# articulatory/articulatory

Hardware: AMD Instinct MI355X
Metric: audio samples/sec (16 kHz) EMA->wav HiFi-CAR, batch 64 (higher is better)
Workload: dtype fp32; 1 GPU; configs[2]: HiFi-CAR (e2w_hifigan_car.yaml generator) 13-dim pitch+EMA -> 16 kHz, batch 64/GPU, 10 s clips, 80 sequential chunks of 25 frames; batch_per_gpu=64, frames=2000, chunk_frames=25, weights=synthetic seed 1234 (articulatory_amd.utils.synth), parallelism=utterance-sharded x1, arithmetic=exact fp32 products (v_mfma_f32_32x32x2_f32), fp32 accumulate, gather=none

## Files before the change

### __graft_entry__.py

```python

import os
import subprocess
import sys

REPO = os.path.dirname(os.path.abspath(__file__))
if REPO not in sys.path:
    sys.path.insert(0, REPO)


def build() -> None:
    csrc = os.path.join(REPO, "articulatory_amd", "csrc")
    subprocess.run(["make", "-C", csrc, f"-j{max(1, min(14, os.cpu_count() or 1))}"], check=True)
    import articulatory_amd
    from articulatory_amd import _native

    lib = _native.load_library()
    for sym in _native.SYMBOLS:
        getattr(lib, sym)
    print("built", _native.LIB_PATH, lib.hificar_version().decode())


def smoke() -> None:
    import numpy as np
    import torch

    from articulatory_amd.models import HiFiGANGenerator
    from articulatory_amd.utils.synth import synth_features, synth_state_dict
# ... 47 lines not shown
```

### articulatory_amd/csrc/hificar.hip

```cpp
#include "hificar_kernels.hip.h"
#include "hificar_launch.h"
#include "hificar_backward.hip.h"
#include "hificar_disc_kernels.hip.h"
#include "hificar_bigru_kernels.hip.h"
#include "hificar_bigru_train_kernels.hip.h"
#include "hificar_xfmr_kernels.hip.h"
#include "hificar_xfmr_attn16.hip.h"
#include "hificar_xfmr_train_kernels.hip.h"
#include "hificar_xfmr_attn16_train.hip.h"
#include "hificar_xfmr_wgrad16.hip.h"

#include "../../include/hificar.h"

#include <algorithm>
#include <queue>
#include <set>
#include <cmath>
#include <cstdarg>
#include <cstdio>
#include <cstring>
#include <functional>
#include <map>
#include <memory>
#include <string>
// ... 51 lines not shown
};

struct PlanKey {
    const ConvLayer* layers[6];
    int nseq, rows, zrep;
    int flags;
    bool operator<(const PlanKey& o) const { return memcmp(this, &o, sizeof(PlanKey)) < 0; }
};

struct ConvPlan {
    ConvShape shape;
    unsigned grid = 0;
    size_t lds = 0;
    std::string name;
    MultiConvParams conv = {};
    PairParams pair = {};
    MergeConvParams merge = {};
    bool merge_wins = false;
};

struct hificar_engine {
    int precision = HIFICAR_PREC_F32;
    int num_cus = 256;
    bool training = false;
    bool profile_detail = false;
    bool use_pair = true;
    bool pair_small = true;
    int mrf_merge = 1;
    int ksplit = 1;
    double mi1_penalty = 1.05;
    int pick_throughput = 0;
    bool shared_chip = false;
    int force_tile[5] = {0, 0, 0, 0, 0};
    std::vector<void*> allocs;
    char* d_zeros = nullptr;
    std::map<PlanKey, ConvPlan> plans;
    struct Arena {
        char* d = nullptr;
        char* h = nullptr;
        size_t cap = 0, used = 0;
    };
    std::vector<Arena> arenas;
    unsigned long long sched_up_seq = 0;
// ... 77 lines not shown
    float* tap_scratch = nullptr;
    size_t tap_scratch_elems = 0;
};

static FILE* g_launch_log = nullptr;
static void read_env_switches(hificar_engine* h) {
    if (const char* e = getenv("HIFICAR_PROFILE_DETAIL")) h->profile_detail = atoi(e) != 0;
    if (const char* e = getenv("HIFICAR_LAUNCH_LOG")) {
        if (!g_launch_log && *e) g_launch_log = fopen(e, "a");
        if (g_launch_log) h->profile_detail = true;
    }
    if (const char* e = getenv("HIFICAR_KSPLIT")) h->ksplit = atoi(e);
    if (const char* e = getenv("HIFICAR_PAIR")) h->use_pair = atoi(e) != 0;
    if (const char* e = getenv("HIFICAR_PAIR_SMALL")) h->pair_small = atoi(e) != 0;
    if (const char* e = getenv("HIFICAR_MRF_MERGE")) h->mrf_merge = atoi(e);
}

struct ProfScope {
    hificar_engine* h;
    hipStream_t s;
    hipEvent_t e0 = nullptr, e1 = nullptr;
    std::string name;
    double flops, bytes;
    ProfScope(hificar_engine* h_, hipStream_t s_, const std::string& n, double f, double b) : h(h_), s(s_), flops(f), bytes(b) {
        if (g_launch_log) {
            fprintf(g_launch_log, "%s\t%.0f\t%.0f\n", n.c_str(), f, b);
            fflush(g_launch_log);
        }
        if (!h->profiling) return;
        name = n;
// ... 359 lines not shown
    if (!L.transposed && L.cin_pad == L.cin && (L.cin == 32 || L.cin == 64) && L.cout == L.cin) {
        if ((rc = pack_w16(h, L, W, L.cin_pad, &L.d_w16c)) != HIFICAR_OK) return rc;
        if ((rc = pack_w32(h, L, W, L.cin_pad, &L.d_w32c)) != HIFICAR_OK) return rc;
    }
    return HIFICAR_OK;
}

hipError_t hificar::conv_launch(const ConvShape& s, const void* params, dim3 grid, size_t lds_bytes, hipStream_t stream) {
    bool handled = false;
    hipError_t e = hipSuccess;
#define HIFICAR_TRY_SET(n)                                                      \
    if (!handled) e = conv_inst_launch_##n(s, params, grid, lds_bytes, stream, &handled); \
    if (handled) return e;
    HIFICAR_TRY_SET(0) HIFICAR_TRY_SET(1) HIFICAR_TRY_SET(2) HIFICAR_TRY_SET(3) HIFICAR_TRY_SET(4)
    HIFICAR_TRY_SET(5) HIFICAR_TRY_SET(6) HIFICAR_TRY_SET(7) HIFICAR_TRY_SET(8) HIFICAR_TRY_SET(9)
    HIFICAR_TRY_SET(10) HIFICAR_TRY_SET(11) HIFICAR_TRY_SET(12)
#undef HIFICAR_TRY_SET
    return hipErrorInvalidValue;
}

hipError_t hificar::conv_set_lds_attributes() {
    hipError_t e = hipSuccess;
#define HIFICAR_ATTR_SET(n) \
    if (e == hipSuccess) e = conv_inst_attrs_##n();
    HIFICAR_ATTR_SET(0) HIFICAR_ATTR_SET(1) HIFICAR_ATTR_SET(2) HIFICAR_ATTR_SET(3) HIFICAR_ATTR_SET(4)
    HIFICAR_ATTR_SET(5) HIFICAR_ATTR_SET(6) HIFICAR_ATTR_SET(7) HIFICAR_ATTR_SET(8) HIFICAR_ATTR_SET(9)
    HIFICAR_ATTR_SET(10) HIFICAR_ATTR_SET(11) HIFICAR_ATTR_SET(12)
#undef HIFICAR_ATTR_SET
    return e;
}

static int engine_open(hificar_engine* h, bool read_env) {
    int dev = 0;
    hipDeviceProp_t prop;
    if (hipGetDevice(&dev) == hipSuccess && hipGetDeviceProperties(&prop, dev) == hipSuccess && prop.multiProcessorCount > 0)
        h->num_cus = prop.multiProcessorCount;
    if (read_env) read_env_switches(h);
    void* z = nullptr;
    HIP_TRY(hipMalloc(&z, 256));
    h->allocs.push_back(z);
    HIP_TRY(hipMemset(z, 0, 256));
    h->d_zeros = static_cast<char*>(z);
// ... 365 lines not shown
            if (!h->xstream_ev) HIP_TRY(hipEventCreateWithFlags(&h->xstream_ev, hipEventDisableTiming));
            HIP_TRY(hipEventRecord(h->xstream_ev, h->last_stream));
            HIP_TRY(hipStreamWaitEvent(stream, h->xstream_ev, 0));
        }
    }
    h->done_valid = false;
    h->last_stream = stream;
    h->have_last_stream = true;
    return HIFICAR_OK;
}

struct TileCfg {
    int MI, WM, WN;
    int KS;
    int NB;
};
static size_t out_buf_bytes(const TileCfg& t) { return (size_t)t.KS * (t.WM * t.MI * 32) * (t.WN * t.NB * 32 + 4) * sizeof(float); }
constexpr int kNumTileCfgs = 15;
static const TileCfg kTileCfgs[kNumTileCfgs] = {{4, 1, 4, 1, 1}, {4, 2, 2, 1, 1}, {4, 4, 1, 1, 1}, {2, 2, 2, 1, 2}, {2, 4, 1, 1, 2},
                                                {2, 1, 4, 1, 2}, {2, 1, 4, 1, 1}, {2, 2, 2, 1, 1}, {2, 4, 1, 1, 1},
                                                {1, 1, 4, 1, 1}, {1, 2, 2, 1, 1}, {1, 4, 1, 1, 1}, {4, 1, 1, 4, 1}, {2, 1, 1, 4, 1}, {1, 1, 1, 4, 1}};

struct ConvIO {
    const char* xs;
    const float* res;
    float* y;
    char* ys;
    const float* mask_src = nullptr;
    float mask_slope = 0.f;
    long long x_seq_bytes = 0;
    int x_row_bytes = 0;
    int x_rows = 0;
    int x_up = 0;
    float x_slope = -1.f;
    const float* x_more[3] = {nullptr, nullptr, nullptr};
    int x_n = 1;
    bool res_relu = false;
};

struct ConvRep {
    int n = 1;
    long long zs_x = 0, zs_w = 0, zs_y = 0, zs_b = 0;
};

static bool tile_admissible(const hificar_engine* h, const ConvLayer* const* layers, int nbr, const TileCfg& t, int halo_all, int nsteps_min) {
    const ConvLayer& L0 = *layers[0];
    const bool f32 = h->precision == HIFICAR_PREC_F32;
    const int TM = t.WM * t.MI * 32, RB = L0.chunk16 * 4;
    if (t.NB == 2 && (f32 || L0.chunk16 == 16)) return false;
    const size_t obuf = (f32 && t.KS == 1) ? 0 : out_buf_bytes(t);
    if (2 * round_up_sz((size_t)(TM + halo_all) * RB, 1024) + obuf > 160 * 1024) return false;
    if (t.NB == 2) {
        bool ok = L0.n_blocks32 >= 2;
        for (int b = 0; b < nbr; ++b) ok = ok && (layers[b]->n_phase == 1 || layers[b]->nb32_per_phase % 2 == 0);
        if (!ok) return false;
    }
    if (t.KS == 4 && (h->ksplit == 0 || nsteps_min < 2)) return false;
    return true;
}

static TileCfg pick_tile(const hificar_engine* h, const ConvLayer* const* layers, int nbr, int nseq, int rows, int zrep, bool merged = false,
                         double* est = nullptr, bool use_force = true) {
    const ConvLayer& L0 = *layers[0];
    const bool f32 = h->precision == HIFICAR_PREC_F32;
    int halo_all = 0;
    for (int b = 0; b < nbr; ++b) halo_all = std::max(halo_all, layers[b]->off_max - layers[b]->off_min);
    TileCfg tc = {1, 4, 1, 1, 1};
    double best = 1e300;
    int nsteps_min = 1 << 30;
    for (int b = 0; b < nbr; ++b) nsteps_min = std::min(nsteps_min, layers[b]->ntaps * (L0.chunk16 / 16));
    if (h->force_tile[0] != 0 && use_force) {
        const TileCfg t = {h->force_tile[0], h->force_tile[1], h->force_tile[2], h->force_tile[3], h->force_tile[4]};
        if (tile_admissible(h, layers, nbr, t, halo_all, nsteps_min) && (!merged || (t.KS == 1 && t.NB == 1))) return t;
    }
    for (int ti = 0; ti < kNumTileCfgs; ++ti) {
        const TileCfg& t = kTileCfgs[ti];
        const int TM = t.WM * t.MI * 32;
        const int chunk = L0.chunk16;
        if (!tile_admissible(h, layers, nbr, t, halo_all, nsteps_min)) continue;
        if (merged && (t.KS != 1 || t.NB != 1)) continue;
        if (!merged && t.KS == 1 && h->ksplit == 2 && nsteps_min >= 2) continue;
        const long long tiles_per_branch = (long long)nseq * ((rows + TM - 1) / TM) * ((L0.n_blocks32 + t.WN * t.NB - 1) / (t.WN * t.NB));
        const int ncls = merged ? 1 : nbr;
        const long long total = tiles_per_branch * ncls * zrep;
        const int G = (int)std::min<long long>(total, h->num_cus);
        const int nchunks = L0.cin_pad / chunk;
        double total_cost = 0.0, heaviest = 0.0, lightest = 1e300, cb[3] = {0.0, 0.0, 0.0};
        for (int b = 0; b < nbr; ++b) {
            const double slab = f32 ? 8 * 64.0 : 3 * 32 / 0.75;
            double c = (double)layers[b]->ntaps * (L0.cin_pad / 16) * slab * t.MI * t.NB + 2500.0 + 400.0 * nchunks;
            if (t.KS == 4) {
                const int steps = layers[b]->ntaps * (chunk / 16);
                c = (double)((steps + 3) / 4) * nchunks * slab * t.MI + 4000.0 + 600.0 * nchunks;
            }
            if (merged) {
                cb[0] += c - (b ? 2500.0 : 0.0);
                continue;
// ... 26 lines not shown
        if (h->pick_throughput > 0 && total >= h->pick_throughput) worst = total_cost / h->num_cus;
        if (t.NB == 2) worst *= f32 ? (t.MI == 4 ? 0.95 : t.MI == 2 ? 0.975 : 1.02) : (t.MI == 2 ? 0.93 : 1.10);
        else if (t.MI < 4) worst *= f32 ? (t.MI == 2 ? 1.02 : h->mi1_penalty) : (t.MI == 2 ? 1.10 : 1.25);
        if (t.KS == 4) worst *= 1.05;
        if (worst < best * 0.98) {
            best = worst;
            tc = t;
        }
    }
    if (est) *est = best;
    return tc;
}

static std::string plan_name(const hificar_engine* h, const ConvShape& s, const ConvLayer& L0, int nbr) {
    static const char* const family[] = {"conv_f32do_kernel", "conv_bf16x3_kernel", "conv_bf16x3nb_kernel", "conv_sk_f32_kernel", "conv_sk_bf16x3_kernel",
                                         "conv_pair_f32_kernel", "conv_pair_bf16x3_kernel", "conv_f32mrg_kernel"};
    char kname[96];
    int n = s.family == kConvSkF32 || s.family == kConvSkBf16x3 ? snprintf(kname, sizeof(kname), "%s<%d,%d>", family[s.family], s.mi, s.nc16)
                                                                : snprintf(kname, sizeof(kname), "%s<%d,%d,%d,%d>", family[s.family], s.mi, s.wm, s.wn, s.nc16);
    if (h->profile_detail) snprintf(kname + n, sizeof(kname) - n, s.family == kConvF32mrg ? "|%s +%d" : "|%s x%d", L0.name.c_str(), nbr);
    return kname;
}

static int build_conv_plan(hificar_engine* h, const ConvLayer* const* layers, int nbr, int nseq, int rows, int zrep, hipStream_t stream, ConvPlan& pl) {
    const ConvLayer& L0 = *layers[0];
    const bool f32 = h->precision == HIFICAR_PREC_F32;
    MultiConvParams& mp = pl.conv;
    const TileCfg tc = pick_tile(h, layers, nbr, nseq, rows, zrep);
    int halo_all = 0;
    for (int b = 0; b < nbr; ++b) halo_all = std::max(halo_all, layers[b]->off_max - layers[b]->off_min);
    const int TM = tc.WM * tc.MI * 32, nc16 = L0.chunk16 / 16;
    const size_t buf_bytes = round_up_sz((size_t)(TM + halo_all) * L0.chunk16 * 4, 1024);
    const bool dout = f32 && tc.KS == 1;
    pl.shape = {dout ? kConvF32do : tc.KS == 4 ? (f32 ? kConvSkF32 : kConvSkBf16x3) : tc.NB == 2 ? kConvBf16x3nb : kConvBf16x3, tc.MI, tc.WM, tc.WN, nc16};
    pl.lds = 2 * buf_bytes + (dout ? 0 : out_buf_bytes(tc));
    mp.buf_bytes = (int)buf_bytes;
    mp.n_branches = nbr;
    mp.nseq_tiles = nseq * ((rows + TM - 1) / TM);
    mp.ngroups = (L0.n_blocks32 + tc.WN * tc.NB - 1) / (tc.WN * tc.NB);
    mp.total_tiles = nbr * zrep * mp.ngroups * mp.nseq_tiles;
    pl.grid = (unsigned)std::min(mp.total_tiles, h->num_cus);
    {
        double wbytes = 0.0;
        for (int b = 0; b < nbr; ++b) wbytes += 4.0 * layers[b]->cin_pad * layers[b]->cout_total * layers[b]->ntaps * zrep;
        const double abytes = 4.0 * nseq * rows * L0.cin_pad * nbr * zrep;
        mp.xcd_order = (mp.total_tiles <= h->num_cus && mp.total_tiles >= 16 && wbytes > 2.0 * abytes) ? 1 : 0;
    }
    mp.stage_cached = mp.ngroups > 2 ? 1 : 0;
    pl.name = plan_name(h, pl.shape, L0, nbr);
    TileLists lists;
    if (mp.total_tiles <= h->num_cus && nbr == 1 && zrep == 1 && mp.ngroups >= 2 && mp.nseq_tiles >= 8 && !h->shared_chip &&
        4.0 * L0.cin_pad * L0.cout_total * L0.ntaps > 6.0e6)
        lists = xcd_block_lists(mp.nseq_tiles, mp.ngroups, h->num_cus);
// ... 103 lines not shown
    pp.in_bytes = (int)round_up_sz((size_t)(TMc + halo_max) * RB, 1024);
    pp.ts_bytes = (int)std::max<size_t>((size_t)(TMc + 16) * RB, (size_t)TMc * (C + 4) * sizeof(float));
    pl.lds = (size_t)pp.in_bytes + pp.ts_bytes;
    if (pl.lds > 160 * 1024) return fail(HIFICAR_E_INVALID, "internal: pair kernel LDS too large (%zu)", pl.lds);
    pl.grid = (unsigned)std::min(tile, h->num_cus);
    pl.shape = {f32 ? kPairF32 : kPairBf16x3, MI, WM, 4 / WM, C / 16};
    pl.name = plan_name(h, pl.shape, *l1[0], nbr);
    if (tile <= (int)pl.grid) return HIFICAR_OK;
    std::vector<double> costs((size_t)tile);
    for (int b = 0; b < nbr; ++b)
        for (int i = pp.tile_start[b]; i < pp.tile_start[b + 1]; ++i) costs[i] = l1[b]->ntaps + l2[b]->ntaps + 2.0;
    return upload_schedule(h, lpt_lists(costs, (int)pl.grid), tile, stream, &pp.sched_start, &pp.sched_tiles);
}

static const ConvPlan* get_plan(hificar_engine* h, const ConvLayer* const* a, const ConvLayer* const* b, int nbr, int nseq, int rows, int zrep,
                                hipStream_t stream, int* rc, bool merged = false) {
    *rc = HIFICAR_OK;
    PlanKey k = {{}, nseq, rows, zrep, (h->precision == HIFICAR_PREC_F32 ? 1 : 0) | (h->training ? 2 : 0) | (h->shared_chip ? 4 : 0) | (b ? 8 : 0) | (merged ? 16 : 0)};
    for (int i = 0; i < nbr; ++i) k.layers[i] = a[i];
    for (int i = 0; b && i < nbr; ++i) k.layers[3 + i] = b[i];
    auto it = h->plans.find(k);
    if (it == h->plans.end()) {
        ConvPlan pl;
        if (h->plans.size() > 20000) *rc = evict_plans(h);
        if (*rc == HIFICAR_OK)
            *rc = merged ? build_merge_plan(h, a, nbr, nseq, rows, stream, pl)
                  : b    ? build_pair_plan(h, a, b, nbr, nseq, rows, stream, pl)
                         : build_conv_plan(h, a, nbr, nseq, rows, zrep, stream, pl);
        if (*rc != HIFICAR_OK) return nullptr;
        it = h->plans.emplace(k, std::move(pl)).first;
    }
    return &it->second;
}

static int launch_conv(hificar_engine* h, const ConvLayer* const* layers, int nbr, int nseq, int rows, const ConvIO* io,
                              float slope_out, const Ragged& rg, hipStream_t stream, const ConvRep& zr = ConvRep()) {
    int rc;
    const ConvPlan* const pl = get_plan(h, layers, nullptr, nbr, nseq, rows, zr.n, stream, &rc);
    if (!pl) return rc;
    const int TM = pl->shape.wm * pl->shape.mi * 32;
    const ConvLayer& L0 = *layers[0];
    const bool f32 = h->precision == HIFICAR_PREC_F32;
    MultiConvParams mp = pl->conv;
    double flops = 0.0, bytes = 0.0;
    for (int b = 0; b < nbr; ++b) {
        const ConvLayer& Lb = *layers[b];
        if (Lb.n_blocks32 != L0.n_blocks32 || Lb.chunk16 != L0.chunk16 || Lb.cin_pad != L0.cin_pad)
            return fail(HIFICAR_E_INVALID, "internal: branch shape mismatch");
        fill_params(mp.p[b], Lb, rows, TM, io[b].res, io[b].y, rg);
        mp.p[b].xs = io[b].xs;
        mp.p[b].ys = io[b].ys;
        if (io[b].x_slope >= 0.f) {
            if (!f32) return fail(HIFICAR_E_INVALID, "internal: pre-activation input rows of %s outside the exact-fp32 layer-by-layer launches", Lb.name.c_str());
            if (io[b].x_n < 1 || io[b].x_n > 4) return fail(HIFICAR_E_INVALID, "internal: %d input streams of %s", io[b].x_n, Lb.name.c_str());
            mp.p[b].act_in = io[b].x_n;
            for (int q = 0; q + 1 < io[b].x_n; ++q) mp.p[b].xs_more[q] = reinterpret_cast<const char*>(io[b].x_more[q]);
            mp.p[b].slope_in = io[b].x_slope;
        }
        if (io[b].res_relu) {
            if (f32 || pl->shape.family == kConvSkBf16x3)
                return fail(HIFICAR_E_INVALID, "internal: pre-activation residual rows of %s outside the dense bf16x3 launches", Lb.name.c_str());
            mp.p[b].res_relu = 1;
        }
        mp.p[b].mask_src = io[b].mask_src;
// ... 11 lines not shown
        mp.p[b].zeros = h->d_zeros;
        mp.p[b].slope_out = slope_out;
        mp.p[b].cout_real = Lb.cout_pad;
        if (f32) mp.p[b].w16 = reinterpret_cast<const bf16x8*>(Lb.d_w32);
        const double pos = (double)nseq * rows;
        flops += 2.0 * pos * Lb.cin * Lb.cout * Lb.K * zr.n;
        bytes += 4.0 * (pos * Lb.cin_pad * (io[b].x_slope >= 0.f ? io[b].x_n : 1) / std::max(1, io[b].x_up) + pos * Lb.cout_total * ((io[b].res ? 1 : 0) + (io[b].y ? 1 : 0) + (io[b].ys ? 1 : 0)) +
                        (double)Lb.cin * Lb.cout * Lb.K);
    }
    mp.zrep = zr.n;
    mp.zs_x = zr.zs_x;
    mp.zs_w = zr.zs_w;
    mp.zs_y = zr.zs_y;
    mp.zs_b = zr.zs_b;
    ProfScope prof(h, stream, pl->name, flops, bytes);
    const hipError_t e = conv_launch(pl->shape, &mp, dim3(pl->grid, 1, 1), pl->lds, stream);
    if (e != hipSuccess) return fail(HIFICAR_E_HIP, "conv launch (%s, %s) failed: %s", L0.name.c_str(), pl->name.c_str(), hipGetErrorString(e));
    return HIFICAR_OK;
}

static int launch_merged(hificar_engine* h, const ConvPlan* pl, const ConvLayer* const* layers, int nbr, int nseq, int rows, const ConvIO* io, char* ys_out,
                         float slope_out, const Ragged& rg, hipStream_t stream) {
    const int TM = pl->shape.wm * pl->shape.mi * 32;
    const ConvLayer& L0 = *layers[0];
    MergeConvParams mp = pl->merge;
    double flops = 0.0, bytes = 0.0;
    const double pos = (double)nseq * rows;
    for (int b = 0; b < nbr; ++b) {
        const ConvLayer& Lb = *layers[b];
        if (Lb.n_blocks32 != L0.n_blocks32 || Lb.chunk16 != L0.chunk16 || Lb.cin_pad != L0.cin_pad || Lb.cout_total != L0.cout_total || Lb.n_phase != 1 ||
            !io[b].res || !io[b].xs || io[b].xs == ys_out)
// ... 962 lines not shown
```

### articulatory_amd/csrc/hificar_conv.hip.h

```cpp
#pragma once
#include <hip/hip_runtime.h>
#include <stdint.h>
#include <type_traits>

namespace hificar {

typedef float f32x2 __attribute__((ext_vector_type(2)));
typedef float f32x4 __attribute__((ext_vector_type(4)));
typedef unsigned u32x4_t __attribute__((ext_vector_type(4)));
typedef float f32x16 __attribute__((ext_vector_type(16)));
typedef __bf16 bf16x4 __attribute__((ext_vector_type(4)));
typedef __bf16 bf16x8 __attribute__((ext_vector_type(8)));

constexpr int kMaxPhase = 8;
constexpr int kMaxTaps = 16;

struct ConvParams {
    const bf16x8* w16;
    const float* bias;
    const float* res;
    const float* mask_src;
    float mask_slope;
    float* y;
    const float* xf;
// ... 28 lines not shown
};

__device__ __forceinline__ int scalar_load_i32(const int* p) {
    int v;
    asm volatile("s_load_dword %0, %1, 0x0\n\ts_waitcnt lgkmcnt(0)" : "=s"(v) : "s"(p) : "memory");
    return v;
}

__device__ __forceinline__ void scalar_load_2i32(const int* p, int& a, int& b) {
    long long v;
    asm volatile("s_load_dwordx2 %0, %1, 0x0\n\ts_waitcnt lgkmcnt(0)" : "=s"(v) : "s"(p) : "memory");
    a = (int)v;
    b = (int)(v >> 32);
}

__device__ __forceinline__ bool is_ragged(const ConvParams& p) { return p.seq_len != nullptr || p.len_const >= 0; }

__device__ __forceinline__ int seq_rows(const ConvParams& p, int seq) {
    if (!is_ragged(p)) return p.L;
    const int n = (p.seq_len ? scalar_load_i32(p.seq_len + __builtin_amdgcn_readfirstlane(seq)) : p.len_const) - p.len_f0;
    return min(max(n, 0), p.len_max) * p.len_mul;
}

template <int NBR>
struct MultiConvParamsN {
    ConvParams p[NBR];
    int n_branches;
    int nseq_tiles;
    int ngroups;
    int total_tiles;
    int buf_bytes;
    const int* sched_start;
    const int* sched_tiles;
    int zrep;
    long long zs_x, zs_w, zs_y, zs_b;
    unsigned long long* trace;
    int xcd_order;
    int stage_cached;
};
struct MultiConvParams : MultiConvParamsN<3> {};
struct MergeConvParams : MultiConvParamsN<4> {};


#ifdef HIFICAR_TRACE
__device__ unsigned long long g_trace_realtime[2][1024];
__device__ unsigned long long g_trace_rt_slots[4][64];
#define HIFICAR_STAMP(slot)                                                                            \
    do {                                                                                               \
        if (mp.trace && lane == 0 && (wave == 0 || wave == kFirstLoader) && (slot) < 64)               \
            mp.trace[((size_t)blockIdx.x * 2 + (wave ? 1 : 0)) * 64 + (slot)] = __builtin_amdgcn_s_memtime(); \
        if (mp.trace && lane == 0 && wave == 0 && ((slot) == 0 || (slot) == 63) && blockIdx.x < 1024)  \
            g_trace_realtime[(slot) == 63][blockIdx.x] = __builtin_amdgcn_s_memrealtime();             \
        if (mp.trace && lane == 0 && wave == 0 && (slot) < 64 && blockIdx.x < 4)                       \
            g_trace_rt_slots[blockIdx.x][(slot)] = __builtin_amdgcn_s_memrealtime();                   \
    } while (0)
// ... 11 lines not shown
        constexpr int lo = NMEM * I / NMFMA, hi = NMEM * (I + 1) / NMFMA;
        constexpr int ds = (hi < NDS ? hi : NDS) - (lo < NDS ? lo : NDS);
        constexpr int vm = (hi - lo) - ds;
        __builtin_amdgcn_sched_group_barrier(0x008, 1, 0);
        if constexpr (ds > 0) __builtin_amdgcn_sched_group_barrier(0x100, ds, 0);
        if constexpr (vm > 0) __builtin_amdgcn_sched_group_barrier(0x020, vm, 0);
        pin_slab_slot<I + 1, NDS, NVMEM, NMFMA>();
    }
}
template <int NDS, int NVMEM, int NMFMA>
__device__ __forceinline__ void pin_slab_step() {
    pin_slab_slot<0, NDS, NVMEM, NMFMA>();
}
__device__ __forceinline__ void lds_barrier() { asm volatile("s_waitcnt lgkmcnt(0)\n\ts_barrier" ::: "memory"); }

template <int MI, int WM, int WN, int NC16, bool F32, int KS = 1, int NB = 1, bool DOUT = false, bool MRG = false, class MP = MultiConvParams>
__device__ __forceinline__ void conv_ws_body(const MP& mp) {
    static_assert(!DOUT || (F32 && KS == 1 && NB == 1), "direct output: exact fp32, dense form, one channel block per wave");
    static_assert(!MRG || DOUT, "branch-summing form: a direct-output kernel");
    static_assert(NB == 1 || (NB == 2 && KS == 1), "one or two channel blocks per MFMA wave");
    static_assert(KS == 1 || (KS == 4 && WM == 1 && WN == 1), "split-K: four waves share one 32-channel block");
    static_assert(KS == 4 || WM * WN == 4 || WM * WN == 8, "4 or 8 MFMA waves per workgroup");
    constexpr int NW = KS == 4 ? 4 : WM * WN;
    constexpr bool kPrimeOnce = DOUT;
    constexpr bool kRowMajorAcc = DOUT;
    constexpr int NTHR = (NW + 4) * 64;
    constexpr int kFirstLoader = NW;
    (void)kFirstLoader;
    static_assert(NC16 == 1 || NC16 == 2 || NC16 == 4, "chunk of 16, 32 or 64 channels");
    constexpr int TM = WM * MI * 32;
    constexpr int CH = NC16 * 16;
    constexpr int RB = CH * 4;
    constexpr int SPR = CH / 4;
    constexpr int LOG_SPR = NC16 == 4 ? 4 : NC16 == 2 ? 3 : 2;
// ... 171 lines not shown
        }
    };
    if (loader) {
        const int lw = wave - NW;
        const int ltid = tid - NW * 64;

        auto dma_item = [&](const Tile& T, int c, int jj) {
            const ConvParams& p = mp.p[T.b];
            const int R = TM + p.halo;
            const int ninstr = (R * SPR + 63) >> 6;
            const int Ls = p.x_rows ? p.x_rows : seq_rows(p, T.seq);
            const int row_bytes = p.x_row_bytes ? p.x_row_bytes : p.cin * 4;
            const char* const xs_z = p.xs + (size_t)T.z * mp.zs_x + (size_t)T.seq * (p.x_seq_bytes ? (size_t)p.x_seq_bytes : (size_t)p.L * p.cin * 4);
            char* dst = smem_b + (jj & 1) * buf_bytes;
            const int c0b = c * CH * 2;
            for (int i = lw; i < ninstr; i += 4) {
                const int n = i * 64 + lane;
                const int r = n >> LOG_SPR;
                const int sl = (n & (SPR - 1)) ^ ((r >> LOG_RPB) & (SPR - 1));
                const int t = T.t0 + p.off_min + r;
                const char* src = p.zeros;
                if (r < R && t >= 0 && t < Ls) {
                    const int ts = p.x_up > 1 ? (int)__umulhi((unsigned)t, p.x_up_rcp) : t;
                    if constexpr (F32) src = xs_z + (size_t)ts * row_bytes + 2 * c0b + sl * 16;
                    else src = xs_z + (size_t)ts * row_bytes + (sl < SPR / 2 ? c0b + sl * 16 : p.cin * 2 + c0b + (sl - SPR / 2) * 16);
                }
                if (mp.stage_cached)
                    __builtin_amdgcn_global_load_lds((const __attribute__((address_space(1))) void*)src,
                                                     (__attribute__((address_space(3))) void*)(dst + i * 1024), 16, 0, 0);
                else
// ... 165 lines not shown
        for (int u = 0; u < NC16; ++u) {
            if constexpr (F32) {
                ad[u][0] = base + (((4 * u + g) ^ swz) << 4);
                ad[u][1] = base + (((4 * u + 2 + g) ^ swz) << 4);
            } else {
                ad[u][0] = base + (((2 * u + g) ^ swz) << 4);
                ad[u][1] = base + (((SPR / 2 + 2 * u + g) ^ swz) << 4);
            }
        }
    };
    auto load_x = [&](frag_t (&xh)[MI], frag_t (&xl)[MI], const int (&ad)[2]) {
#pragma unroll
        for (int mi = 0; mi < MI; ++mi) {
            xh[mi] = *reinterpret_cast<const frag_t*>(smem_b + ad[0] + mi * 32 * RB);
            xl[mi] = *reinterpret_cast<const frag_t*>(smem_b + ad[1] + mi * 32 * RB);
        }
    };
    auto mfma_step = [&](const frag_t (&xh)[MI], const frag_t (&xl)[MI], const frag_t (&wh)[NB], const frag_t (&wl)[NB]) {
        if constexpr (F32) {
#pragma unroll
            for (int s4 = 0; s4 < 4; ++s4)
#pragma unroll
                for (int q = 0; q < NB; ++q)
#pragma unroll
                    for (int mi = 0; mi < MI; ++mi) {
                        if constexpr (kRowMajorAcc) acc[q][mi] = __builtin_amdgcn_mfma_f32_32x32x2f32(xh[mi][s4], wh[q][s4], acc[q][mi], 0, 0, 0);
                        else acc[q][mi] = __builtin_amdgcn_mfma_f32_32x32x2f32(wh[q][s4], xh[mi][s4], acc[q][mi], 0, 0, 0);
                    }
#pragma unroll
            for (int s4 = 0; s4 < 4; ++s4)
// ... 305 lines not shown
                for (int mi = 0; mi < MI; ++mi)
#pragma unroll
                    for (int r = 0; r < 16; ++r) acc[q][mi][r] = 0.f;
        }
        float bias_l = 0.f;
        float bias_b[4] = {0.f, 0.f, 0.f, 0.f};
        (void)bias_b;
        const bool last_branch = !MRG || T.b == mp.n_branches - 1;
        if constexpr (MRG) {
            if (last_branch) {
#pragma unroll
                for (int b = 0; b < 4; ++b)
                    if (b < mp.n_branches) bias_b[b] = mp.p[b].bias[(nb < p.n_blocks32 ? nb : 0) * 32 + li];
            }
        } else if constexpr (kRowMajorAcc) bias_l = bias_of(T);

        for (int c = 0; c < nchunks; ++c, ++j) {
            HIFICAR_STAMP(1 + 3 * j);
            lds_barrier();
            HIFICAR_STAMP(2 + 3 * j);
            if constexpr (!kPrimeOnce) {
                if (!active) continue;
            }
            const int buf_off = (j & 1) * buf_bytes;
            int ad[NC16][2];
            addr_set(buf_off, roff0, ad);
            if constexpr (NC16 % 2 == 0) {
                frag_t x0h[MI], x0l[MI], x1h[MI], x1l[MI];
                load_x(x0h, x0l, ad[0]);
                for (int t = 0; t < ntaps; ++t) {
                    const bool last_tap = t + 1 == ntaps;
                    int adn[NC16][2];
                    addr_set(buf_off, roff0 + (last_tap ? t : t + 1) * tap_step, adn);
                    if (groups_left == 0) {
                        wp = wp_next;
                        if constexpr (NB == 2) wp2 = wp_next + wst_next;
                        groups_left = groups_next;
                    }
                    --groups_left;
// ... 64 lines not shown
                        *reinterpret_cast<f32x4*>(&O[(wave_row0 + mi * 32 + li) * OP + (wn * NB + b2) * 32 + 8 * q + 4 * g]) = v;
                    }
        }
    }
    lds_barrier();
    HIFICAR_STAMP(62);
    if constexpr (!DOUT) {
        if (last >= 0) write_out(decode(tile_of(last)), tid, NTHR);
    }
    HIFICAR_STAMP(63);
}

template <int MI, int WM, int WN, int NC16>
__global__ __launch_bounds__((WM * WN + 4) * 64) void conv_f32do_kernel(const MultiConvParams mp) {
    conv_ws_body<MI, WM, WN, NC16, true, 1, 1, true>(mp);
}

template <int MI, int WM, int WN, int NC16>
__global__ __launch_bounds__((WM * WN + 4) * 64) void conv_f32mrg_kernel(const MergeConvParams mp) {
    conv_ws_body<MI, WM, WN, NC16, true, 1, 1, true, true>(mp);
}

template <int MI, int WM, int WN, int NC16>
__global__ __launch_bounds__((WM * WN + 4) * 64) void conv_bf16x3_kernel(const MultiConvParams mp) {
    conv_ws_body<MI, WM, WN, NC16, false>(mp);
}

template <int MI, int WM, int WN, int NC16>
__global__ __launch_bounds__((WM * WN + 4) * 64) void conv_bf16x3nb_kernel(const MultiConvParams mp) {
    conv_ws_body<MI, WM, WN, NC16, false, 1, 2>(mp);
// ... 484 lines not shown
```

### articulatory_amd/csrc/hificar_conv_inst.hip

```cpp
#include "hificar_conv.hip.h"
#include "hificar_launch.h"

#ifndef HIFICAR_INST_SET
#error "compile with -DHIFICAR_INST_SET=0..12"
#endif

namespace hificar {

#define HIFICAR_TILES9(X, nc) X(4, 1, 4, nc) X(4, 2, 2, nc) X(4, 4, 1, nc) X(2, 1, 4, nc) X(2, 2, 2, nc) X(2, 4, 1, nc) X(1, 1, 4, nc) X(1, 2, 2, nc) X(1, 4, 1, nc)

#if HIFICAR_INST_SET == 0
#define FAMILY kConvF32do
#define KERNEL conv_f32do_kernel
#define PARAMS MultiConvParams
#define SHAPES(X) HIFICAR_TILES9(X, 1)
#elif HIFICAR_INST_SET == 1
#define FAMILY kConvF32do
#define KERNEL conv_f32do_kernel
#define PARAMS MultiConvParams
#define SHAPES(X) HIFICAR_TILES9(X, 2)
#elif HIFICAR_INST_SET == 2
#define FAMILY kConvF32do
#define KERNEL conv_f32do_kernel
#define PARAMS MultiConvParams
// ... 28 lines not shown
#endif
#define THREADS(wm, wn) 512
#define PARAMS MultiConvParams
#define SHAPES(X) X(1, 1, 1, 1) X(2, 1, 1, 1) X(4, 1, 1, 1) X(1, 1, 1, 2) X(2, 1, 1, 2) X(4, 1, 1, 2) X(1, 1, 1, 4) X(2, 1, 1, 4) X(4, 1, 1, 4)
#elif HIFICAR_INST_SET >= 10 && HIFICAR_INST_SET <= 12
#define FAMILY kConvF32mrg
#define KERNEL conv_f32mrg_kernel
#define PARAMS MergeConvParams
#if HIFICAR_INST_SET == 10
#define SHAPES(X) HIFICAR_TILES9(X, 1)
#elif HIFICAR_INST_SET == 11
#define SHAPES(X) HIFICAR_TILES9(X, 2)
#else
#define SHAPES(X) HIFICAR_TILES9(X, 4)
#endif
#elif HIFICAR_INST_SET == 9
#define PARAMS PairParams
#define THREADS(wm, wn) 512
#else
#error "HIFICAR_INST_SET out of range"
#endif

#ifndef KERNEL_PTR
#define KERNEL_PTR(mi, wm, wn, nc) (KERNEL<mi, wm, wn, nc>)
#endif
#ifndef THREADS
#define THREADS(wm, wn) ((wm * wn + 4) * 64)
#endif

#define HIFICAR_CAT_(a, b) a##b
// ... 67 lines not shown
```

### articulatory_amd/csrc/hificar_launch.h

```cpp
#pragma once
#include <hip/hip_runtime.h>

namespace hificar {

struct MultiConvParams;
struct MergeConvParams;
struct PairParams;

enum ConvFamily {
    kConvF32do = 0,
    kConvBf16x3 = 1,
    kConvBf16x3nb = 2,
    kConvSkF32 = 3,
    kConvSkBf16x3 = 4,
    kPairF32 = 5,
    kPairBf16x3 = 6,
    kConvF32mrg = 7,
};

struct ConvShape {
    int family, mi, wm, wn, nc16;
};

hipError_t conv_launch(const ConvShape& s, const void* params, dim3 grid, size_t lds_bytes, hipStream_t stream);
hipError_t conv_set_lds_attributes();

#define HIFICAR_N_INST_SETS 13
#define HIFICAR_DECL_SET(n)                                                                                                              \
    hipError_t conv_inst_launch_##n(const ConvShape& s, const void* params, dim3 grid, size_t lds, hipStream_t stream, bool* handled); \
    hipError_t conv_inst_attrs_##n();
HIFICAR_DECL_SET(0) HIFICAR_DECL_SET(1) HIFICAR_DECL_SET(2) HIFICAR_DECL_SET(3) HIFICAR_DECL_SET(4)
HIFICAR_DECL_SET(5) HIFICAR_DECL_SET(6) HIFICAR_DECL_SET(7) HIFICAR_DECL_SET(8) HIFICAR_DECL_SET(9)
HIFICAR_DECL_SET(10) HIFICAR_DECL_SET(11) HIFICAR_DECL_SET(12)
#undef HIFICAR_DECL_SET

}
```

Before: 40.19 million samples/s.

## Add dense-row conv kernel packing multiple short sequences into one M tile

```diff
diff --git a/__graft_entry__.py b/__graft_entry__.py
--- a/__graft_entry__.py
+++ b/__graft_entry__.py
@@ -10,7 +10,7 @@
 
 def build() -> None:
     csrc = os.path.join(REPO, "articulatory_amd", "csrc")
-    subprocess.run(["make", "-C", csrc, f"-j{max(1, min(14, os.cpu_count() or 1))}"], check=True)
+    subprocess.run(["make", "-C", csrc, f"-j{max(1, min(15, os.cpu_count() or 1))}"], check=True)
     import articulatory_amd
     from articulatory_amd import _native
 
diff --git a/articulatory_amd/csrc/hificar.hip b/articulatory_amd/csrc/hificar.hip
--- a/articulatory_amd/csrc/hificar.hip
+++ b/articulatory_amd/csrc/hificar.hip
@@ -89,6 +89,7 @@
     size_t lds = 0;
     std::string name;
     MultiConvParams conv = {};
+    int dense_gap = -1;
     PairParams pair = {};
     MergeConvParams merge = {};
     bool merge_wins = false;
@@ -102,6 +103,7 @@
     bool use_pair = true;
     bool pair_small = true;
     int mrf_merge = 1;
+    int dense_rows = 1;
     int ksplit = 1;
     double mi1_penalty = 1.05;
     int pick_throughput = 0;
@@ -209,6 +211,7 @@
     if (const char* e = getenv("HIFICAR_PAIR")) h->use_pair = atoi(e) != 0;
     if (const char* e = getenv("HIFICAR_PAIR_SMALL")) h->pair_small = atoi(e) != 0;
     if (const char* e = getenv("HIFICAR_MRF_MERGE")) h->mrf_merge = atoi(e);
+    if (const char* e = getenv("HIFICAR_DENSE_ROWS")) h->dense_rows = atoi(e);
 }
 
 struct ProfScope {
@@ -598,7 +601,7 @@
     if (handled) return e;
     HIFICAR_TRY_SET(0) HIFICAR_TRY_SET(1) HIFICAR_TRY_SET(2) HIFICAR_TRY_SET(3) HIFICAR_TRY_SET(4)
     HIFICAR_TRY_SET(5) HIFICAR_TRY_SET(6) HIFICAR_TRY_SET(7) HIFICAR_TRY_SET(8) HIFICAR_TRY_SET(9)
-    HIFICAR_TRY_SET(10) HIFICAR_TRY_SET(11) HIFICAR_TRY_SET(12)
+    HIFICAR_TRY_SET(10) HIFICAR_TRY_SET(11) HIFICAR_TRY_SET(12) HIFICAR_TRY_SET(13)
 #undef HIFICAR_TRY_SET
     return hipErrorInvalidValue;
 }
@@ -609,7 +612,7 @@
     if (e == hipSuccess) e = conv_inst_attrs_##n();
     HIFICAR_ATTR_SET(0) HIFICAR_ATTR_SET(1) HIFICAR_ATTR_SET(2) HIFICAR_ATTR_SET(3) HIFICAR_ATTR_SET(4)
     HIFICAR_ATTR_SET(5) HIFICAR_ATTR_SET(6) HIFICAR_ATTR_SET(7) HIFICAR_ATTR_SET(8) HIFICAR_ATTR_SET(9)
-    HIFICAR_ATTR_SET(10) HIFICAR_ATTR_SET(11) HIFICAR_ATTR_SET(12)
+    HIFICAR_ATTR_SET(10) HIFICAR_ATTR_SET(11) HIFICAR_ATTR_SET(12) HIFICAR_ATTR_SET(13)
 #undef HIFICAR_ATTR_SET
     return e;
 }
@@ -1005,6 +1008,7 @@
     int MI, WM, WN;
     int KS;
     int NB;
+    bool dense = false;
 };
 static size_t out_buf_bytes(const TileCfg& t) { return (size_t)t.KS * (t.WM * t.MI * 32) * (t.WN * t.NB * 32 + 4) * sizeof(float); }
 constexpr int kNumTileCfgs = 15;
@@ -1034,13 +1038,13 @@
     long long zs_x = 0, zs_w = 0, zs_y = 0, zs_b = 0;
 };
 
-static bool tile_admissible(const hificar_engine* h, const ConvLayer* const* layers, int nbr, const TileCfg& t, int halo_all, int nsteps_min) {
+static bool tile_admissible(const hificar_engine* h, const ConvLayer* const* layers, int nbr, const TileCfg& t, int halo_all, int nsteps_min, int gap_rows = 0) {
     const ConvLayer& L0 = *layers[0];
     const bool f32 = h->precision == HIFICAR_PREC_F32;
     const int TM = t.WM * t.MI * 32, RB = L0.chunk16 * 4;
     if (t.NB == 2 && (f32 || L0.chunk16 == 16)) return false;
     const size_t obuf = (f32 && t.KS == 1) ? 0 : out_buf_bytes(t);
-    if (2 * round_up_sz((size_t)(TM + halo_all) * RB, 1024) + obuf > 160 * 1024) return false;
+    if (2 * round_up_sz((size_t)(TM + halo_all + gap_rows) * RB, 1024) + obuf > 160 * 1024) return false;
     if (t.NB == 2) {
         bool ok = L0.n_blocks32 >= 2;
         for (int b = 0; b < nbr; ++b) ok = ok && (layers[b]->n_phase == 1 || layers[b]->nb32_per_phase % 2 == 0);
@@ -1050,8 +1054,23 @@
     return true;
 }
 
+static int dense_rows_mode(const hificar_engine* h) {
+    return (h->ksplit != 1 || !h->use_pair || h->precision != HIFICAR_PREC_F32 || h->training || h->shared_chip) ? 0 : h->dense_rows;
+}
+static int dense_gap(const ConvLayer* const* layers, int nbr) {
+    int gap = 0;
+    for (int b = 0; b < nbr; ++b) gap = std::max(gap, std::max(layers[b]->off_max, -layers[b]->off_min));
+    return gap;
+}
+static int dense_gap_rows(int TM, int rows, int gap) { return ((TM + rows - 1) / rows + 1) * gap; }
+static bool dense_shape(const hificar_engine* h, const ConvLayer* const* layers, int nbr, const TileCfg& t, int nseq, int rows, int halo_all, int nsteps_min) {
+    const int TM = t.WM * t.MI * 32;
+    return t.KS == 1 && t.NB == 1 && t.MI >= 2 && layers[0]->chunk16 == 64 && nseq >= 2 && rows < TM &&
+           tile_admissible(h, layers, nbr, t, halo_all, nsteps_min, dense_gap_rows(TM, rows, dense_gap(layers, nbr)));
+}
+
 static TileCfg pick_tile(const hificar_engine* h, const ConvLayer* const* layers, int nbr, int nseq, int rows, int zrep, bool merged = false,
-                         double* est = nullptr, bool use_force = true) {
+                         double* est = nullptr, bool use_force = true, int dense_mode = 0) {
     const ConvLayer& L0 = *layers[0];
     const bool f32 = h->precision == HIFICAR_PREC_F32;
     int halo_all = 0;
@@ -1062,16 +1081,28 @@
     for (int b = 0; b < nbr; ++b) nsteps_min = std::min(nsteps_min, layers[b]->ntaps * (L0.chunk16 / 16));
     if (h->force_tile[0] != 0 && use_force) {
         const TileCfg t = {h->force_tile[0], h->force_tile[1], h->force_tile[2], h->force_tile[3], h->force_tile[4]};
-        if (tile_admissible(h, layers, nbr, t, halo_all, nsteps_min) && (!merged || (t.KS == 1 && t.NB == 1))) return t;
-    }
-    for (int ti = 0; ti < kNumTileCfgs; ++ti) {
-        const TileCfg& t = kTileCfgs[ti];
+        if (tile_admissible(h, layers, nbr, t, halo_all, nsteps_min) && (!merged || (t.KS == 1 && t.NB == 1))) {
+            TileCfg tf = t;
+            if (dense_mode && !merged && dense_shape(h, layers, nbr, t, nseq, rows, halo_all, nsteps_min))
+                tf.dense = dense_mode == 2 || pick_tile(h, layers, nbr, nseq, rows, zrep, false, nullptr, false, dense_mode).dense;
+            return tf;
+        }
+    }
+    if (merged) dense_mode = 0;
+    bool any_dense = false;
+    for (int ti = 0; ti < kNumTileCfgs && dense_mode == 2; ++ti)
+        any_dense = any_dense || dense_shape(h, layers, nbr, kTileCfgs[ti], nseq, rows, halo_all, nsteps_min);
+    for (int tf = 0; tf < 2 * kNumTileCfgs; ++tf) {
+        TileCfg t = kTileCfgs[tf >> 1];
+        t.dense = (tf & 1) != 0;
         const int TM = t.WM * t.MI * 32;
         const int chunk = L0.chunk16;
+        if (t.dense ? !(dense_mode && dense_shape(h, layers, nbr, t, nseq, rows, halo_all, nsteps_min)) : any_dense) continue;
         if (!tile_admissible(h, layers, nbr, t, halo_all, nsteps_min)) continue;
         if (merged && (t.KS != 1 || t.NB != 1)) continue;
         if (!merged && t.KS == 1 && h->ksplit == 2 && nsteps_min >= 2) continue;
-        const long long tiles_per_branch = (long long)nseq * ((rows + TM - 1) / TM) * ((L0.n_blocks32 + t.WN * t.NB - 1) / (t.WN * t.NB));
+        const long long row_tiles = t.dense ? ((long long)nseq * rows + TM - 1) / TM : (long long)nseq * ((rows + TM - 1) / TM);
+        const long long tiles_per_branch = row_tiles * ((L0.n_blocks32 + t.WN * t.NB - 1) / (t.WN * t.NB));
         const int ncls = merged ? 1 : nbr;
         const long long total = tiles_per_branch * ncls * zrep;
         const int G = (int)std::min<long long>(total, h->num_cus);
@@ -1128,29 +1159,33 @@
 
 static std::string plan_name(const hificar_engine* h, const ConvShape& s, const ConvLayer& L0, int nbr) {
     static const char* const family[] = {"conv_f32do_kernel", "conv_bf16x3_kernel", "conv_bf16x3nb_kernel", "conv_sk_f32_kernel", "conv_sk_bf16x3_kernel",
-                                         "conv_pair_f32_kernel", "conv_pair_bf16x3_kernel", "conv_f32mrg_kernel"};
+                                         "conv_pair_f32_kernel", "conv_pair_bf16x3_kernel", "conv_f32mrg_kernel", "conv_f32dd_kernel"};
     char kname[96];
     int n = s.family == kConvSkF32 || s.family == kConvSkBf16x3 ? snprintf(kname, sizeof(kname), "%s<%d,%d>", family[s.family], s.mi, s.nc16)
                                                                 : snprintf(kname, sizeof(kname), "%s<%d,%d,%d,%d>", family[s.family], s.mi, s.wm, s.wn, s.nc16);
-    if (h->profile_detail) snprintf(kname + n, sizeof(kname) - n, s.family == kConvF32mrg ? "|%s +%d" : "|%s x%d", L0.name.c_str(), nbr);
+    if (h->profile_detail)
+        snprintf(kname + n, sizeof(kname) - n, s.family == kConvF32mrg ? "|%s +%d" : s.family == kConvF32dd ? "|%s d%d" : "|%s x%d", L0.name.c_str(), nbr);
     return kname;
 }
 
-static int build_conv_plan(hificar_engine* h, const ConvLayer* const* layers, int nbr, int nseq, int rows, int zrep, hipStream_t stream, ConvPlan& pl) {
+static int build_conv_plan(hificar_engine* h, const ConvLayer* const* layers, int nbr, int nseq, int rows, int zrep, bool dense_ok, hipStream_t stream,
+                           ConvPlan& pl) {
     const ConvLayer& L0 = *layers[0];
     const bool f32 = h->precision == HIFICAR_PREC_F32;
     MultiConvParams& mp = pl.conv;
-    const TileCfg tc = pick_tile(h, layers, nbr, nseq, rows, zrep);
+    const TileCfg tc = pick_tile(h, layers, nbr, nseq, rows, zrep, false, nullptr, true, dense_ok ? dense_rows_mode(h) : 0);
     int halo_all = 0;
     for (int b = 0; b < nbr; ++b) halo_all = std::max(halo_all, layers[b]->off_max - layers[b]->off_min);
     const int TM = tc.WM * tc.MI * 32, nc16 = L0.chunk16 / 16;
-    const size_t buf_bytes = round_up_sz((size_t)(TM + halo_all) * L0.chunk16 * 4, 1024);
+    if (tc.dense) pl.dense_gap = dense_gap(layers, nbr);
+    const size_t buf_bytes = round_up_sz((size_t)(TM + halo_all + (tc.dense ? dense_gap_rows(TM, rows, pl.dense_gap) : 0)) * L0.chunk16 * 4, 1024);
     const bool dout = f32 && tc.KS == 1;
-    pl.shape = {dout ? kConvF32do : tc.KS == 4 ? (f32 ? kConvSkF32 : kConvSkBf16x3) : tc.NB == 2 ? kConvBf16x3nb : kConvBf16x3, tc.MI, tc.WM, tc.WN, nc16};
+    pl.shape = {tc.dense ? kConvF32dd : dout ? kConvF32do : tc.KS == 4 ? (f32 ? kConvSkF32 : kConvSkBf16x3) : tc.NB == 2 ? kConvBf16x3nb : kConvBf16x3,
+                tc.MI, tc.WM, tc.WN, nc16};
     pl.lds = 2 * buf_bytes + (dout ? 0 : out_buf_bytes(tc));
     mp.buf_bytes = (int)buf_bytes;
     mp.n_branches = nbr;
-    mp.nseq_tiles = nseq * ((rows + TM - 1) / TM);
+    mp.nseq_tiles = tc.dense ? (int)(((long long)nseq * rows + TM - 1) / TM) : nseq * ((rows + TM - 1) / TM);
     mp.ngroups = (L0.n_blocks32 + tc.WN * tc.NB - 1) / (tc.WN * tc.NB);
     mp.total_tiles = nbr * zrep * mp.ngroups * mp.nseq_tiles;
     pl.grid = (unsigned)std::min(mp.total_tiles, h->num_cus);
@@ -1284,9 +1319,10 @@
 }
 
 static const ConvPlan* get_plan(hificar_engine* h, const ConvLayer* const* a, const ConvLayer* const* b, int nbr, int nseq, int rows, int zrep,
-                                hipStream_t stream, int* rc, bool merged = false) {
+                                hipStream_t stream, int* rc, bool merged = false, bool dense_ok = false) {
     *rc = HIFICAR_OK;
-    PlanKey k = {{}, nseq, rows, zrep, (h->precision == HIFICAR_PREC_F32 ? 1 : 0) | (h->training ? 2 : 0) | (h->shared_chip ? 4 : 0) | (b ? 8 : 0) | (merged ? 16 : 0)};
+    PlanKey k = {{}, nseq, rows, zrep, (h->precision == HIFICAR_PREC_F32 ? 1 : 0) | (h->training ? 2 : 0) | (h->shared_chip ? 4 : 0) | (b ? 8 : 0) | (merged ? 16 : 0) |
+                                       (dense_ok ? 32 : 0)};
     for (int i = 0; i < nbr; ++i) k.layers[i] = a[i];
     for (int i = 0; b && i < nbr; ++i) k.layers[3 + i] = b[i];
     auto it = h->plans.find(k);
@@ -1296,28 +1332,41 @@
         if (*rc == HIFICAR_OK)
             *rc = merged ? build_merge_plan(h, a, nbr, nseq, rows, stream, pl)
                   : b    ? build_pair_plan(h, a, b, nbr, nseq, rows, stream, pl)
-                         : build_conv_plan(h, a, nbr, nseq, rows, zrep, stream, pl);
+                         : build_conv_plan(h, a, nbr, nseq, rows, zrep, dense_ok, stream, pl);
         if (*rc != HIFICAR_OK) return nullptr;
         it = h->plans.emplace(k, std::move(pl)).first;
     }
     return &it->second;
+}
+
+static bool dense_rows_allowed(const hificar_engine* h, const ConvLayer* const* layers, int nbr, int nseq, int rows, const ConvIO* io, const Ragged& rg,
+                               const ConvRep& zr) {
+    if (dense_rows_mode(h) == 0 || zr.n != 1 || nseq < 2 || rg.seq_len || rg.const_len >= 0) return false;
+    for (int b = 0; b < nbr; ++b) {
+        const ConvIO& q = io[b];
+        if (q.x_slope >= 0.f || q.x_row_bytes != 0 || q.x_rows != 0 || q.x_up > 1 || q.mask_src || q.res_relu) return false;
+        if (q.x_seq_bytes != 0 && q.x_seq_bytes != (long long)rows * layers[b]->cin_pad * 4) return false;
+    }
+    const long long P = (long long)rows + dense_gap(layers, nbr);
+    return ((long long)nseq * P + 4096) * P < (1LL << 32);
 }
 
 static int launch_conv(hificar_engine* h, const ConvLayer* const* layers, int nbr, int nseq, int rows, const ConvIO* io,
                               float slope_out, const Ragged& rg, hipStream_t stream, const ConvRep& zr = ConvRep()) {
     int rc;
-    const ConvPlan* const pl = get_plan(h, layers, nullptr, nbr, nseq, rows, zr.n, stream, &rc);
+    const ConvPlan* const pl = get_plan(h, layers, nullptr, nbr, nseq, rows, zr.n, stream, &rc, false, dense_rows_allowed(h, layers, nbr, nseq, rows, io, rg, zr));
     if (!pl) return rc;
     const int TM = pl->shape.wm * pl->shape.mi * 32;
     const ConvLayer& L0 = *layers[0];
     const bool f32 = h->precision == HIFICAR_PREC_F32;
+    const bool dense = pl->shape.family == kConvF32dd;
     MultiConvParams mp = pl->conv;
     double flops = 0.0, bytes = 0.0;
     for (int b = 0; b < nbr; ++b) {
         const ConvLayer& Lb = *layers[b];
         if (Lb.n_blocks32 != L0.n_blocks32 || Lb.chunk16 != L0.chunk16 || Lb.cin_pad != L0.cin_pad)
             return fail(HIFICAR_E_INVALID, "internal: branch shape mismatch");
-        fill_params(mp.p[b], Lb, rows, TM, io[b].res, io[b].y, rg);
+        fill_params(mp.p[b], Lb, dense ? nseq * rows : rows, TM, io[b].res, io[b].y, rg);
         mp.p[b].xs = io[b].xs;
         mp.p[b].ys = io[b].ys;
         if (io[b].x_slope >= 0.f) {
@@ -1359,7 +1408,20 @@
     mp.zs_y = zr.zs_y;
     mp.zs_b = zr.zs_b;
     ProfScope prof(h, stream, pl->name, flops, bytes);
-    const hipError_t e = conv_launch(pl->shape, &mp, dim3(pl->grid, 1, 1), pl->lds, stream);
+    hipError_t e;
+    if (dense) {
+        DenseConvParams dp;
+        static_cast<MultiConvParamsN<3>&>(dp) = mp;
+        dp.dense_L = rows;
+        dp.dense_gap = pl->dense_gap;
+        dp.dense_nseq = nseq;
+        dp.dense_extra = dense_gap_rows(TM, rows, pl->dense_gap);
+        dp.dense_rcp_L = (unsigned)(0x100000000ull / (unsigned)rows + 1u);
+        dp.dense_rcp_P = (unsigned)(0x100000000ull / (unsigned)(rows + pl->dense_gap) + 1u);
+        e = conv_launch(pl->shape, &dp, dim3(pl->grid, 1, 1), pl->lds, stream);
+    } else {
+        e = conv_launch(pl->shape, &mp, dim3(pl->grid, 1, 1), pl->lds, stream);
+    }
     if (e != hipSuccess) return fail(HIFICAR_E_HIP, "conv launch (%s, %s) failed: %s", L0.name.c_str(), pl->name.c_str(), hipGetErrorString(e));
     return HIFICAR_OK;
 }
diff --git a/articulatory_amd/csrc/hificar_conv.hip.h b/articulatory_amd/csrc/hificar_conv.hip.h
--- a/articulatory_amd/csrc/hificar_conv.hip.h
+++ b/articulatory_amd/csrc/hificar_conv.hip.h
@@ -66,6 +66,8 @@
     b = (int)(v >> 32);
 }
 
+__device__ __forceinline__ unsigned dense_div(unsigned x, int d, unsigned rcp) { return d == 1 ? x : __umulhi(x, rcp); }
+
 __device__ __forceinline__ bool is_ragged(const ConvParams& p) { return p.seq_len != nullptr || p.len_const >= 0; }
 
 __device__ __forceinline__ int seq_rows(const ConvParams& p, int seq) {
@@ -91,6 +93,10 @@
     int stage_cached;
 };
 struct MultiConvParams : MultiConvParamsN<3> {};
+struct DenseConvParams : MultiConvParamsN<3> {
+    int dense_L, dense_gap, dense_nseq, dense_extra;
+    unsigned dense_rcp_L, dense_rcp_P;
+};
 struct MergeConvParams : MultiConvParamsN<4> {};
 
 
@@ -132,10 +138,11 @@
 }
 __device__ __forceinline__ void lds_barrier() { asm volatile("s_waitcnt lgkmcnt(0)\n\ts_barrier" ::: "memory"); }
 
-template <int MI, int WM, int WN, int NC16, bool F32, int KS = 1, int NB = 1, bool DOUT = false, bool MRG = false, class MP = MultiConvParams>
+template <int MI, int WM, int WN, int NC16, bool F32, int KS = 1, int NB = 1, bool DOUT = false, bool MRG = false, class MP = MultiConvParams, bool DENSE = false>
 __device__ __forceinline__ void conv_ws_body(const MP& mp) {
     static_assert(!DOUT || (F32 && KS == 1 && NB == 1), "direct output: exact fp32, dense form, one channel block per wave");
     static_assert(!MRG || DOUT, "branch-summing form: a direct-output kernel");
+    static_assert(!DENSE || (DOUT && !MRG), "dense rows: the plain direct-output kernel");
     static_assert(NB == 1 || (NB == 2 && KS == 1), "one or two channel blocks per MFMA wave");
     static_assert(KS == 1 || (KS == 4 && WM == 1 && WN == 1), "split-K: four waves share one 32-channel block");
     static_assert(KS == 4 || WM * WN == 4 || WM * WN == 8, "4 or 8 MFMA waves per workgroup");
@@ -337,6 +344,31 @@
             const char* const xs_z = p.xs + (size_t)T.z * mp.zs_x + (size_t)T.seq * (p.x_seq_bytes ? (size_t)p.x_seq_bytes : (size_t)p.L * p.cin * 4);
             char* dst = smem_b + (jj & 1) * buf_bytes;
             const int c0b = c * CH * 2;
+            if constexpr (DENSE) {
+                const int Ld = mp.dense_L, P = Ld + mp.dense_gap;
+                const int Rd = R + mp.dense_extra;
+                const int nin = (Rd * SPR + 63) >> 6;
+                const int q0 = T.t0 + mp.dense_gap * (int)dense_div((unsigned)T.t0, Ld, mp.dense_rcp_L) + p.off_min;
+                const size_t seq_bytes = p.x_seq_bytes ? (size_t)p.x_seq_bytes : (size_t)Ld * row_bytes;
+                const char* const xs_d = p.xs + (size_t)T.z * mp.zs_x;
+                for (int i = lw; i < nin; i += 4) {
+                    const int n = i * 64 + lane;
+                    const int r = n >> LOG_SPR;
+                    const int sl = (n & (SPR - 1)) ^ ((r >> LOG_RPB) & (SPR - 1));
+                    const int q = q0 + r;
+                    const int s = (int)dense_div((unsigned)max(q, 0), P, mp.dense_rcp_P);
+                    const int t = q - s * P;
+                    const char* src = p.zeros;
+                    if (r < Rd && q >= 0 && t < Ld && s < mp.dense_nseq) src = xs_d + (size_t)s * seq_bytes + (size_t)t * row_bytes + 2 * c0b + sl * 16;
+                    if (mp.stage_cached)
+                        __builtin_amdgcn_global_load_lds((const __attribute__((address_space(1))) void*)src,
+                                                         (__attribute__((address_space(3))) void*)(dst + i * 1024), 16, 0, 0);
+                    else
+                        __builtin_amdgcn_global_load_lds((const __attribute__((address_space(1))) void*)src,
+                                                         (__attribute__((address_space(3))) void*)(dst + i * 1024), 16, 0, 2);
+                }
+                return;
+            }
             for (int i = lw; i < ninstr; i += 4) {
                 const int n = i * 64 + lane;
                 const int r = n >> LOG_SPR;
@@ -532,6 +564,29 @@
         for (int mi = 0; mi < MI; ++mi) {
             xh[mi] = *reinterpret_cast<const frag_t*>(smem_b + ad[0] + mi * 32 * RB);
             xl[mi] = *reinterpret_cast<const frag_t*>(smem_b + ad[1] + mi * 32 * RB);
+        }
+    };
+    int gap_rows[MI];
+#pragma unroll
+    for (int mi = 0; mi < MI; ++mi) gap_rows[mi] = 0;
+    auto addr_set_d = [&](int buf_off, int roff, int (&ad)[MI][NC16][2]) {
+#pragma unroll
+        for (int mi = 0; mi < MI; ++mi) {
+            const int r0 = wave_row0 + mi * 32 + li + gap_rows[mi] + roff;
+            const int swz = (r0 >> LOG_RPB) & (SPR - 1);
+            const int base = buf_off + r0 * RB;
+#pragma unroll
+            for (int u = 0; u < NC16; ++u) {
+                ad[mi][u][0] = base + (((4 * u + g) ^ swz) << 4);
+                ad[mi][u][1] = base + (((4 * u + 2 + g) ^ swz) << 4);
+            }
+        }
+    };
+    auto load_x_d = [&](frag_t (&xh)[MI], frag_t (&xl)[MI], const int (&ad)[MI][NC16][2], int u) {
+#pragma unroll
+        for (int mi = 0; mi < MI; ++mi) {
+            xh[mi] = *reinterpret_cast<const frag_t*>(smem_b + ad[mi][u][0]);
+            xl[mi] = *reinterpret_cast<const frag_t*>(smem_b + ad[mi][u][1]);
         }
     };
     auto mfma_step = [&](const frag_t (&xh)[MI], const frag_t (&xl)[MI], const frag_t (&wh)[NB], const frag_t (&wl)[NB]) {
@@ -867,6 +922,12 @@
                     if (b < mp.n_branches) bias_b[b] = mp.p[b].bias[(nb < p.n_blocks32 ? nb : 0) * 32 + li];
             }
         } else if constexpr (kRowMajorAcc) bias_l = bias_of(T);
+        if constexpr (DENSE) {
+            const unsigned s0 = dense_div((unsigned)T.t0, mp.dense_L, mp.dense_rcp_L);
+#pragma unroll
+            for (int mi = 0; mi < MI; ++mi)
+                gap_rows[mi] = mp.dense_gap * (int)(dense_div((unsigned)(T.t0 + wave_row0 + mi * 32 + li), mp.dense_L, mp.dense_rcp_L) - s0);
+        }
 
         for (int c = 0; c < nchunks; ++c, ++j) {
             HIFICAR_STAMP(1 + 3 * j);
@@ -876,6 +937,40 @@
                 if (!active) continue;
             }
             const int buf_off = (j & 1) * buf_bytes;
+            if constexpr (DENSE) {
+                static_assert(!DENSE || NC16 % 2 == 0, "dense rows: even chunk sizes");
+                int ad[MI][NC16][2];
+                addr_set_d(buf_off, roff0, ad);
+                frag_t x0h[MI], x0l[MI], x1h[MI], x1l[MI];
+                load_x_d(x0h, x0l, ad, 0);
+                for (int t = 0; t < ntaps; ++t) {
+                    const bool last_tap = t + 1 == ntaps;
+                    int adn[MI][NC16][2];
+                    addr_set_d(buf_off, roff0 + (last_tap ? t : t + 1) * tap_step, adn);
+                    if (groups_left == 0) {
+                        wp = wp_next;
+                        groups_left = groups_next;
+                    }
+                    --groups_left;
+#pragma unroll
+                    for (int u = 0; u < NC16; u += 2) {
+                        load_x_d(x1h, x1l, ad, u + 1);
+                        slab_step(x0h, x0l, u);
+                        if (u + 2 < NC16) load_x_d(x0h, x0l, ad, u + 2);
+                        else load_x_d(x0h, x0l, adn, 0);
+                        slab_step(x1h, x1l, u + 1);
+                    }
+                    wp += NC16 * 128;
+#pragma unroll
+                    for (int mi = 0; mi < MI; ++mi)
+#pragma unroll
+                        for (int u = 0; u < NC16; ++u) {
+                            ad[mi][u][0] = adn[mi][u][0];
+                            ad[mi][u][1] = adn[mi][u][1];
+                        }
+                }
+                continue;
+            }
             int ad[NC16][2];
             addr_set(buf_off, roff0, ad);
             if constexpr (NC16 % 2 == 0) {
@@ -970,6 +1065,11 @@
 template <int MI, int WM, int WN, int NC16>
 __global__ __launch_bounds__((WM * WN + 4) * 64) void conv_f32do_kernel(const MultiConvParams mp) {
     conv_ws_body<MI, WM, WN, NC16, true, 1, 1, true>(mp);
+}
+
+template <int MI, int WM, int WN, int NC16>
+__global__ __launch_bounds__((WM * WN + 4) * 64) void conv_f32dd_kernel(const DenseConvParams mp) {
+    conv_ws_body<MI, WM, WN, NC16, true, 1, 1, true, false, DenseConvParams, true>(mp);
 }
 
 template <int MI, int WM, int WN, int NC16>
diff --git a/articulatory_amd/csrc/hificar_conv_inst.hip b/articulatory_amd/csrc/hificar_conv_inst.hip
--- a/articulatory_amd/csrc/hificar_conv_inst.hip
+++ b/articulatory_amd/csrc/hificar_conv_inst.hip
@@ -2,7 +2,7 @@
 #include "hificar_launch.h"
 
 #ifndef HIFICAR_INST_SET
-#error "compile with -DHIFICAR_INST_SET=0..12"
+#error "compile with -DHIFICAR_INST_SET=0..13"
 #endif
 
 namespace hificar {
@@ -66,6 +66,11 @@
 #else
 #define SHAPES(X) HIFICAR_TILES9(X, 4)
 #endif
+#elif HIFICAR_INST_SET == 13
+#define FAMILY kConvF32dd
+#define KERNEL conv_f32dd_kernel
+#define PARAMS DenseConvParams
+#define SHAPES(X) X(4, 1, 4, 4) X(4, 2, 2, 4) X(4, 4, 1, 4) X(2, 1, 4, 4) X(2, 2, 2, 4) X(2, 4, 1, 4)
 #elif HIFICAR_INST_SET == 9
 #define PARAMS PairParams
 #define THREADS(wm, wn) 512
diff --git a/articulatory_amd/csrc/hificar_launch.h b/articulatory_amd/csrc/hificar_launch.h
--- a/articulatory_amd/csrc/hificar_launch.h
+++ b/articulatory_amd/csrc/hificar_launch.h
@@ -5,6 +5,7 @@
 
 struct MultiConvParams;
 struct MergeConvParams;
+struct DenseConvParams;
 struct PairParams;
 
 enum ConvFamily {
@@ -16,6 +17,7 @@
     kPairF32 = 5,
     kPairBf16x3 = 6,
     kConvF32mrg = 7,
+    kConvF32dd = 8,
 };
 
 struct ConvShape {
@@ -25,13 +27,13 @@
 hipError_t conv_launch(const ConvShape& s, const void* params, dim3 grid, size_t lds_bytes, hipStream_t stream);
 hipError_t conv_set_lds_attributes();
 
-#define HIFICAR_N_INST_SETS 13
+#define HIFICAR_N_INST_SETS 14
 #define HIFICAR_DECL_SET(n)                                                                                                              \
     hipError_t conv_inst_launch_##n(const ConvShape& s, const void* params, dim3 grid, size_t lds, hipStream_t stream, bool* handled); \
     hipError_t conv_inst_attrs_##n();
 HIFICAR_DECL_SET(0) HIFICAR_DECL_SET(1) HIFICAR_DECL_SET(2) HIFICAR_DECL_SET(3) HIFICAR_DECL_SET(4)
 HIFICAR_DECL_SET(5) HIFICAR_DECL_SET(6) HIFICAR_DECL_SET(7) HIFICAR_DECL_SET(8) HIFICAR_DECL_SET(9)
-HIFICAR_DECL_SET(10) HIFICAR_DECL_SET(11) HIFICAR_DECL_SET(12)
+HIFICAR_DECL_SET(10) HIFICAR_DECL_SET(11) HIFICAR_DECL_SET(12) HIFICAR_DECL_SET(13)
 #undef HIFICAR_DECL_SET
 
 }
```

After: 40.42 million samples/s (median of 6 runs). No clear change (+0.6%).
